# stefantaubert/waveglow

Hardware: AMD Instinct MI355X
Metric: audio samples/sec/GPU (22.05 kHz) WaveGlow-256 infer; real-time factor (higher is better)
Workload: dtype f16 MFMA operands, f32 accumulate/flow state, fp16 I/O; 1 GPU; configs[1]: 256ch WaveGlow.infer, batch=16/GPU mels 80x864, fp16 I/O, sigma=0.6; parallelism=utterance-sharded x1, no collective

## Files before the change

waveglow_amd/csrc/kernels.hip:

```cpp
#include "wg_common.h"

#include <cstdlib>
#include <type_traits>

namespace wg {

typedef _Float16 half8 __attribute__((ext_vector_type(8)));
typedef _Float16 half4 __attribute__((ext_vector_type(4)));
typedef float f32x16 __attribute__((ext_vector_type(16)));
typedef float f32x4 __attribute__((ext_vector_type(4)));

#define WG_GPTR(p) ((const __attribute__((address_space(1))) void*)(p))
#define WG_LPTR(p) ((__attribute__((address_space(3))) void*)(p))

__device__ __forceinline__ float load_io(const void* p, size_t i, int f16) {
  return f16 ? (float)((const _Float16*)p)[i] : ((const float*)p)[i];
}

__device__ __forceinline__ float gate_act(float u, float v) {
  const float e1 = __builtin_amdgcn_exp2f(__builtin_amdgcn_fmed3f(u, -60.0f, 60.0f));
  const float t = 1.0f + __builtin_amdgcn_exp2f(v);
  return (e1 - 1.0f) * __builtin_amdgcn_rcpf(fmaf(e1, t, t));
}

__device__ __forceinline__ void gate_act3(float u, float v, float& th, float& sg, float& ac) {
  const float e1 = __builtin_amdgcn_exp2f(__builtin_amdgcn_fmed3f(u, -60.0f, 60.0f));
  const float t = 1.0f + __builtin_amdgcn_exp2f(__builtin_amdgcn_fmed3f(v, -60.0f, 60.0f));
  const float r = __builtin_amdgcn_rcpf(fmaf(e1, t, t));
  ac = fmaf(e1, r, -r);
  sg = fmaf(e1, r, r);
  th = ac * t;
}

__device__ __forceinline__ void glds16(const void* sbase, unsigned voff, unsigned lds_addr) {
  unsigned keep;
  asm volatile("s_mov_b32 %0, m0\n\ts_mov_b32 m0, %3\n\ts_nop 2\n\tglobal_load_lds_dwordx4 %1, %2\n\ts_mov_b32 m0, %0"
               : "=&s"(keep) : "v"(voff), "s"(sbase), "s"(lds_addr) : "memory");
}
template <int OFF>
__device__ __forceinline__ void gload16(half8& dst, const void* sbase, unsigned voff) {
  asm volatile("s_nop 4\n\tglobal_load_dwordx4 %0, %1, %2 offset:%3" : "=v"(dst) : "v"(voff), "s"(sbase), "i"(OFF) : "memory");
}

#ifdef WG_STAMPS
#define WG_STAMP(i)                                                                              \
  do {                                                                                           \
    __builtin_amdgcn_sched_barrier(0);                                                           \
    unsigned long long _t;                                                                       \
    asm volatile("s_memtime %0\n\ts_waitcnt lgkmcnt(0)" : "=s"(_t)::"memory");                   \
    if (a.stamps && HAS_RES && tid == 0) a.stamps[(size_t)tile * 8 + (i)] = _t;                        \
    __builtin_amdgcn_sched_barrier(0);                                                           \
  } while (0)
#else
#define WG_STAMP(i) do {} while (0)
#endif

constexpr int kTilesPerWG = 2;


__device__ __forceinline__ void mfma16_acc(f32x4& c, const half8& a, const half8& b) {
  c = __builtin_amdgcn_mfma_f32_16x16x32_f16(a, b, c, 0, 0, 0);
}

template <int C> struct WnCfg {
  static constexpr int NW = (C >= 256) ? 8 : C / 32;
  static constexpr int BN = (C >= 512) ? 64 : 128;
};

template <int N> __device__ __forceinline__ void wait_vm() {
  asm volatile("s_waitcnt vmcnt(%0)" :: "i"(N) : "memory");
  __builtin_amdgcn_sched_barrier(0);
}

template <int C, int NW, int BN, bool HAS_RES, int TPW, int CX, int MODE = 0, int NTAPS = 3, bool HAS_COND = true, bool DEEP = false, bool M16 = false>
__global__ void __launch_bounds__(NW * 64) wn_layer_kernel(const WnLayerArgs a) {
  constexpr bool TR = MODE == 1;
  constexpr bool PLAIN = MODE >= 2;
  constexpr int MB = C / (32 * NW);
  constexpr int MT = PLAIN ? MB : 2 * MB;
  constexpr int NTHREADS = NW * 64;
  constexpr int NT = BN / 32;
  constexpr int CC = CX;
  constexpr int NKX = NTAPS * CC;
  constexpr int BT_BYTES = BN * 128;
  constexpr int ACT_ROW = 2 * C + 16;
  constexpr int K2 = C / 16;
  constexpr int NG = BN * 8 / NTHREADS;
  constexpr int NAH = MT * 2;
  constexpr bool DEFER = (MB == 1);
  static_assert(BN * 8 % NTHREADS == 0 && MB >= 1 && MB <= 2 && NKX >= 1 && (NTAPS == 1 || NTAPS == 3), "tile geometry");
  constexpr bool Q2L = !M16 && DEFER && !DEEP && (NG + NT - 1) / NT == 1 && NT >= NG + MT;
  static_assert(!M16 || (MODE == 0 && MB == 1 && DEFER && !DEEP && NT >= 2), "16x16x32 variant");
  constexpr bool A0G = MODE == 0 && CX == 1 && NTAPS == 1;
  static_assert(!DEEP || (MODE == 0 && DEFER && HAS_COND && MT <= NT && NG <= NT && ((NKX >= 4 && NKX % 2 == 0) || NKX == 1)), "deep prefetch variant");
  static_assert(MODE == 0 || (TPW == 1 && CX == ((MODE == 2 || MODE == 4) ? 2 : 1) * (C / 64)) || (MODE == 3 && CX == 1), "training variants");

  extern __shared__ __attribute__((aligned(16))) char smem[];
  char* const sB = smem;
  char* const sActs = MODE == 4 ? smem : smem + 2 * BT_BYTES;

  const int tid = threadIdx.x;
  const int wave = __builtin_amdgcn_readfirstlane(tid >> 6);
  int lane = tid & 63, ln = lane & 31, lh = lane >> 5;

  unsigned pvoff[NG];
  int pchunk[NG];
  int swB;
  int l15 = lane & 15, l4 = lane >> 4;
  unsigned a_voff;
  auto set_lane_ids = [&]() {
    int t = tid;
    asm volatile("" : "+v"(t));
    lane = t & 63;
    ln = lane & 31;
    lh = lane >> 5;
    swB = M16 ? (lane >> 1) & 7 : (ln >> 1) & 7;
    l15 = lane & 15;
    l4 = lane >> 4;
    a_voff = lane * 16;
#pragma unroll
    for (int i = 0; i < NG; ++i) {
      const int idx = i * NTHREADS + t;
      const int row = idx >> 3, pc = idx & 7;
      pchunk[i] = pc ^ ((row >> 1) & 7);
      pvoff[i] = row * 128 + (pchunk[i] << 4);
    }
  };
  set_lane_ids();
  const unsigned sB_addr = (unsigned)(size_t)WG_LPTR(sB);
  const int R = a.g.R, Rp = a.g.Rp, Fp = a.g.Fp, M = a.M;
  const int nK = NKX + (HAS_COND ? a.n_cond_steps : 0);
  const int mel_rows_per_utt = a.g.T + 6;

  auto xstep_src = [&](int p, int jt, int ks) -> const char* {
    const int tap = ks / CC, cc = ks - tap * CC;
    const int pp = p + (tap - NTAPS / 2) * a.dil;
    const int row = kRowPad + (pp & 31) * Rp + a.row0 + jt * BN + (pp >> 5);
    return (const char*)(a.x_tap + ((size_t)cc * R + row) * 64);
  };
  auto sp_src = [&](int p, int jt, int s_) -> const char* {
    const int row = kRowPad + p * Rp + a.row0 + jt * BN;
    return (const char*)(a.sp + ((size_t)s_ * R + row) * 64);
  };
  int mrow[NG];
  auto cond_voff = [&](int s, int i) -> unsigned {
    const int k0 = s * 64 + pchunk[i] * 8;
    const int j = (k0 >= M) + (k0 >= 2 * M) + (k0 >= 3 * M);
    return (unsigned)(((mrow[i] - j) * M + (k0 - j * M)) * 2);
  };
  auto stage_B_piece = [&](int p, int jt, int ks, int bufsel, int i) {
    const unsigned lds = __builtin_amdgcn_readfirstlane(sB_addr + bufsel * BT_BYTES + (i * NTHREADS + wave * 64) * 16);
    if constexpr (A0G) {
      if (ks < NKX) {
        const int row = (i * NTHREADS + tid) >> 3, lc = pchunk[i];
        const int pp = p + ((lc < 3 ? lc : 1) - 1) * a.dil;
        const unsigned prow = (unsigned)(kRowPad + (pp & 31) * Rp + a.row0 + jt * BN + (pp >> 5) + row);
        glds16(a.x_tap, prow * 128u + (lc < 3 ? 0u : (unsigned)lc * 16u), lds);
        return;
      }
    }
    if (ks < NKX) glds16(xstep_src(p, jt, ks), pvoff[i], lds);
    else if constexpr (MODE != 0) glds16(sp_src(p, jt, ks - NKX), pvoff[i], lds);
    else glds16(a.melT, cond_voff(ks - NKX, i), lds);
  };
  auto read_B = [&](const char* buf, int nt, int k16) -> half8 {
    const int n = nt * 32 + ln;
    const int c = (k16 * 2 + lh) ^ swB;
    return *(const half8*)(buf + n * 128 + c * 16);
  };
  auto read_B16 = [&](const char* buf, int g, int nt) -> half8 {
    const int n = (NT * (g & 1) + nt) * 16 + l15;
    const int c = (4 * (g >> 1) + l4) ^ swB;
    return *(const half8*)(buf + n * 128 + c * 16);
  };
  const char* wA1c_p = nullptr;
  auto load_Aq = [&](int ks, int g, int mt, half8& dst) {
    const char* base = ks < NKX ? (const char*)a.wA1 : wA1c_p;
    const int kl = ks < NKX ? ks : ks - NKX;
    const char* p = base + ((size_t)(2 * kl + (g >> 1)) * NW + wave) * (NAH * 1024) + (mt * 2 + (g & 1)) * 1024;
    gload16<0>(dst, p, a_voff);
  };
  auto load_A16 = [&](int ks, int s_, int m, half8& dst) {
    const char* base = ks < NKX ? (const char*)a.wA1 : wA1c_p;
    const int kl = ks < NKX ? ks : ks - NKX;
    gload16<0>(dst, base + ((size_t)(2 * kl + s_) * NW + wave) * (NAH * 1024) + m * 1024, a_voff);
  };
  int tile_b0 = 0;
  const bool fp_ge_bn = Fp >= BN;
  auto column_of = [&](int rr, int p, int& b, int& t) -> bool {
    int rem = rr - tile_b0 * Fp;
    b = tile_b0;
    if (fp_ge_bn) {
      if (rem >= Fp) { rem -= Fp; ++b; }
    } else {
      const int qd = rem / Fp;
      b += qd;
      rem -= qd * Fp;
    }
    const int fq = rem - a.g.Gf;
    t = fq * 32 + p;
    if (!(b < a.g.B && fq >= 0 && fq < a.g.F && t < a.g.L)) return false;
    return a.g.frames == nullptr || t < 32 * a.g.frames[b];
  };

  int tile, tile_end;
  const int tile_step = gridDim.x >> 3;
  int run_start, run_quarter = 0;
  {
    const int bid = blockIdx.x, ntl = a.n_tiles;
    const int xcd = bid & 7, idx = bid >> 3;
    const int qq = ntl >> 3, r = ntl & 7;
    const int start = xcd < r ? xcd * (qq + 1) : r * (qq + 1) + (xcd - r) * qq;
    tile_end = start + (xcd < r ? qq + 1 : qq);
    tile = start + idx;
    run_start = start;
    if (((tile_end - start) & 3) == 0) run_quarter = (tile_end - start) >> 2;
  }
  auto tile_of = [&](int t) { return run_quarter ? run_start + ((t - run_start) & 3) * run_quarter + ((t - run_start) >> 2) : t; };

  half8 q[4][MT];
  int par = 0;
  if (tile < tile_end) {
    const int t0 = tile_of(tile), p0 = t0 / a.tiles_per_phase;
#pragma unroll
    for (int i = 0; i < NG; ++i) stage_B_piece(p0, t0 - p0 * a.tiles_per_phase, 0, 0, i);
  }
  float* const sBias = (float*)(sActs + BN * ACT_ROW);
  if constexpr (!PLAIN) {
    for (int i = tid; i < 2 * C; i += NTHREADS) sBias[i] = a.bias1[i];
    if constexpr (HAS_RES)
      for (int i = tid; i < C; i += NTHREADS) sBias[2 * C + i] = a.bias2[i];
    uint4* const sW = (uint4*)(sBias + 3 * C);
    for (int i = tid; i < (C / 32) * 64; i += NTHREADS) sW[i] = ((const uint4*)a.wEs)[i];
  }
  __syncthreads();

#pragma unroll
  for (int it = 0; it < TPW; ++it, tile += tile_step) {
    if (tile >= tile_end) break;
    if (it > 0) set_lane_ids();
    const int tile_m = tile_of(tile);
    const int p = tile_m / a.tiles_per_phase;
    const int jt = tile_m - p * a.tiles_per_phase;
    const int rr0 = a.row0 + jt * BN;
    tile_b0 = rr0 / Fp;
    const int r0 = kRowPad + p * Rp + rr0;
    const int next_tile = tile + tile_step;
    wA1c_p = (const char*)a.wA1c + (MODE != 0 ? (size_t)0 : (size_t)p * (2 * a.n_cond_steps) * NW * (NAH * 1024));
    half8 Q[DEEP ? 2 : 1][4][MT];
    if constexpr (DEEP) {
#pragma unroll
      for (int g = 0; g < 4; ++g)
#pragma unroll
        for (int mt = 0; mt < MT; ++mt) load_Aq(0, g, mt, Q[0][g][mt]);
#pragma unroll
      for (int g = 0; g < 2; ++g)
#pragma unroll
        for (int mt = 0; mt < MT; ++mt) load_Aq(1, g, mt, Q[DEEP ? 1 : 0][g][mt]);
    } else {
#pragma unroll
      for (int g = 0; g < (Q2L || M16 ? 2 : 3); ++g)
#pragma unroll
        for (int mt = 0; mt < MT; ++mt) {
          if constexpr (M16) load_A16(0, 0, 2 * g + mt, q[g][mt]);
          else load_Aq(0, g, mt, q[g][mt]);
        }
    }
    if constexpr (MODE == 0) {
#pragma unroll
      for (int i = 0; i < NG; ++i) {
        int b, t;
        const int rr = rr0 + ((i * NTHREADS + tid) >> 3);
        const bool ok = column_of(rr, p, b, t);
        mrow[i] = ok ? 3 + b * mel_rows_per_utt + 3 + (t >> 5) : 3;
      }
    }
    unsigned vmask = 0;
#pragma unroll
    for (int nt = 0; nt < NT; ++nt) {
      int cb, ct;
      vmask |= column_of(rr0 + nt * 32 + ln, p, cb, ct) ? (1u << nt) : 0u;
    }
    WG_STAMP(0);
    f32x16 acc[MT][NT];
    f32x4 acc4[M16 ? MT : 1][M16 ? NT : 1][4];
    auto acc_at = [&](int mt, int nt, int e) -> float {
      if constexpr (M16) return acc4[mt][nt][e >> 2][e & 3];
      else return acc[mt][nt][e];
    };
#pragma unroll
    for (int mt = 0; mt < MT; ++mt) {
      f32x16 v;
      if constexpr (PLAIN) {
#pragma unroll
        for (int j = 0; j < 16; ++j) v[j] = 0.0f;
      } else {
        const int row0 = (mt < MB ? 0 : C) + (wave * MB + (mt < MB ? mt : mt - MB)) * 32;
        const float4* bp = (const float4*)(sBias + row0 + 4 * (M16 ? l4 : lh));
#pragma unroll
        for (int g = 0; g < 4; ++g) {
          const float4 q4 = bp[M16 ? 4 * (g >> 1) : 2 * g];
          v[4 * g] = q4.x; v[4 * g + 1] = q4.y; v[4 * g + 2] = q4.z; v[4 * g + 3] = q4.w;
        }
      }
#pragma unroll
      for (int nt = 0; nt < NT; ++nt) {
        if constexpr (M16) {
#pragma unroll
          for (int e = 0; e < 4; ++e) acc4[mt][nt][e] = f32x4{v[4 * e], v[4 * e + 1], v[4 * e + 2], v[4 * e + 3]};
        } else {
          acc[mt][nt] = v;
        }
      }
    }

    constexpr bool PIPE = !PLAIN && HAS_RES && MB == 1;
    constexpr bool RES_A0 = A0G && wn_res_a0(C);
    half8 a2r[PIPE ? K2 : 1];
    wait_vm<DEEP ? 3 * MT : 0>();
    __builtin_amdgcn_s_barrier();
    __builtin_amdgcn_sched_barrier(0);
    WG_STAMP(1);
    constexpr int LPS = (MT + NT - 1) / NT;
    constexpr int GPS = (NG + NT - 1) / NT;
    half8 bf[2][NT];
    constexpr bool PRIO = NW == 8 && ((BN == 128 && ((MODE == 0 && CX == C / 64) || MODE == 1)) || (C == 512 && MODE == 0 && CX == C / 64));
    auto prio_set = [&](int hi_grp) {
      if (hi_grp == 1)
        asm volatile("s_cmp_lt_u32 %0, 4\n\ts_cbranch_scc1 .Lpa%=\n\ts_setprio 1\n\ts_branch .Lpb%=\n.Lpa%=:\n\ts_setprio 0\n.Lpb%=:" :: "s"(wave) : "memory", "scc");
      else
        asm volatile("s_cmp_lt_u32 %0, 4\n\ts_cbranch_scc1 .Lpa%=\n\ts_setprio 0\n\ts_branch .Lpb%=\n.Lpa%=:\n\ts_setprio 1\n.Lpb%=:" :: "s"(wave) : "memory", "scc");
    };
    auto mfma_col = [&](int g, int nt) {
      if constexpr (M16) {
        const int t16 = NT * (g & 1) + nt;
#pragma unroll
        for (int m = 0; m < 4; ++m) {
          mfma16_acc(acc4[m >> 1][t16 >> 1][2 * (m & 1) + (t16 & 1)], q[2 * (g >> 1) + (m >> 1)][m & 1], bf[g & 1][nt]);
        }
      } else {
#pragma unroll
        for (int mt = 0; mt < MT; ++mt) {
          acc[mt][nt] = __builtin_amdgcn_mfma_f32_32x32x16_f16(q[g][mt], bf[g & 1][nt], acc[mt][nt], 0, 0, 0);
        }
      }
    };
    auto kstep = [&](auto more_tag, auto ncond_tag, auto first_tag, int ks) {
      constexpr bool more = decltype(more_tag)::value;
      constexpr bool ncond = decltype(ncond_tag)::value;
      constexpr bool first = decltype(first_tag)::value;
      const char* buf = sB + ((ks + par) & 1) * BT_BYTES;
      const char* src_next = nullptr;
      if constexpr (more && !ncond) src_next = xstep_src(p, jt, ks + 1);
      if constexpr (more && ncond && MODE != 0) src_next = sp_src(p, jt, ks + 1 - NKX);
      const unsigned lds_next = sB_addr + ((ks + 1 + par) & 1) * BT_BYTES + wave * 1024;
#pragma unroll
      for (int nt = 0; nt < NT; ++nt) bf[0][nt] = M16 ? read_B16(buf, 0, nt) : read_B(buf, nt, 0);
      __builtin_amdgcn_sched_barrier(0);
      auto dma_slot = [&](int nt) {
        if constexpr (more) {
#pragma unroll
          for (int i = nt * GPS; i < (nt + 1) * GPS && i < NG; ++i) {
            const unsigned lds = __builtin_amdgcn_readfirstlane(lds_next + i * NTHREADS * 16);
            if constexpr (ncond && MODE == 0) glds16(a.melT, cond_voff(ks + 1 - NKX, i), lds);
            else glds16(src_next, pvoff[i], lds);
          }
        }
      };
      if constexpr (PRIO) {
        prio_set(1);
        __builtin_amdgcn_sched_barrier(0);
      }
      if constexpr (DEFER) {
#pragma unroll
        for (int nt = 0; nt < NT; ++nt) {
          if constexpr (!first) mfma_col(3, nt);
          __builtin_amdgcn_sched_barrier(0);
          dma_slot(nt);
          if constexpr (Q2L) {
            if (nt >= NG && nt - NG < MT) load_Aq(ks, 2, nt - NG, q[2][nt - NG]);
          }
          __builtin_amdgcn_sched_barrier(0);
        }
      }
#pragma unroll
      for (int g = 0; g < (DEFER ? 3 : 4); ++g) {
        if constexpr (M16) {
          if (g == 0) wait_vm<more ? NG : 0>();
          if (g == 2) wait_vm<0>();
        } else {
        if (g == 1) wait_vm<more ? 2 * MT + NG : 2 * MT>();
        if (g == 2) wait_vm<Q2L ? (more ? 2 * MT : MT) : (more ? NG + 2 * MT : MT)>();
        if (g == 3) wait_vm<more ? 2 * MT : 0>();
        }
#pragma unroll
        for (int nt = 0; nt < NT; ++nt) {
          mfma_col(g, nt);
          __builtin_amdgcn_sched_barrier(0);
          if (g < 3) bf[(g + 1) & 1][nt] = M16 ? read_B16(buf, g + 1, nt) : read_B(buf, nt, g + 1);
          if (!DEFER && g == 0) dma_slot(nt);
          if constexpr (M16) {
            constexpr int LP16 = (4 + NT - 1) / NT;
            if (g == 0 || (g == 2 && more)) {
#pragma unroll
              for (int m = nt * LP16; m < (nt + 1) * LP16 && m < 4; ++m)
                load_A16(g == 0 ? ks : ks + 1, g == 0 ? 1 : 0, m, q[(g == 0 ? 2 : 0) + (m >> 1)][m & 1]);
            }
          } else if (g == 0 || more) {
#pragma unroll
            for (int mt = nt * LPS; mt < (nt + 1) * LPS && mt < MT; ++mt)
              load_Aq(g == 0 ? ks : ks + 1, (g + 3) & 3, mt, q[(g + 3) & 3][mt]);
          }
          if constexpr (PRIO) {
            if (g == 0 && nt == NT - 1) prio_set(0);
          }
          __builtin_amdgcn_sched_barrier(0);
        }
      }
      if constexpr (more) {
        if constexpr (DEFER && !Q2L && !M16) {
#pragma unroll
          for (int mt = 0; mt < MT; ++mt) load_Aq(ks + 1, 2, mt, q[2][mt]);
        }
        asm volatile("s_waitcnt vmcnt(%0) lgkmcnt(0)" :: "i"(M16 ? 4 : Q2L ? MT : 2 * MT) : "memory");
        __builtin_amdgcn_s_barrier();
        __builtin_amdgcn_sched_barrier(0);
      }
    };
    auto kstep_d = [&](auto par_tag, auto more_tag, auto more2_tag, auto ncond_tag, auto first_tag, int ks) {
      constexpr int P = DEEP ? decltype(par_tag)::value : 0, PO = DEEP ? 1 - P : 0;
      constexpr bool more = decltype(more_tag)::value, more2 = decltype(more2_tag)::value;
      constexpr bool ncond = decltype(ncond_tag)::value, first = decltype(first_tag)::value;
      const char* buf = sB + ((ks + par) & 1) * BT_BYTES;
      const char* src_next = nullptr;
      if constexpr (more && !ncond) src_next = xstep_src(p, jt, ks + 1);
      const unsigned lds_next = sB_addr + ((ks + 1 + par) & 1) * BT_BYTES + wave * 1024;
#pragma unroll
      for (int nt = 0; nt < NT; ++nt) bf[0][nt] = read_B(buf, nt, 0);
      __builtin_amdgcn_sched_barrier(0);
#pragma unroll
      for (int nt = 0; nt < NT; ++nt) {
        if constexpr (!first) {
#pragma unroll
          for (int mt = 0; mt < MT; ++mt)
            acc[mt][nt] = __builtin_amdgcn_mfma_f32_32x32x16_f16(Q[PO][3][mt], bf[1][nt], acc[mt][nt], 0, 0, 0);
        }
        __builtin_amdgcn_sched_barrier(0);
        if constexpr (more) {
          if (nt < NG) {
            const unsigned lds = __builtin_amdgcn_readfirstlane(lds_next + nt * NTHREADS * 16);
            if constexpr (ncond) glds16(a.melT, cond_voff(ks + 1 - NKX, nt), lds);
            else glds16(src_next, pvoff[nt], lds);
          }
          if (nt == NT - 1) {
#pragma unroll
            for (int mt = 0; mt < MT; ++mt) load_Aq(ks + 1, 2, mt, Q[PO][2][mt]);
          }
        }
        __builtin_amdgcn_sched_barrier(0);
      }
#pragma unroll
      for (int g = 0; g < 3; ++g) {
#pragma unroll
        for (int nt = 0; nt < NT; ++nt) {
#pragma unroll
          for (int mt = 0; mt < MT; ++mt)
            acc[mt][nt] = __builtin_amdgcn_mfma_f32_32x32x16_f16(Q[P][g][mt], bf[g & 1][nt], acc[mt][nt], 0, 0, 0);
          __builtin_amdgcn_sched_barrier(0);
          bf[(g + 1) & 1][nt] = read_B(buf, nt, g + 1);
          if (nt < MT) {
            if (g == 0 && more) load_Aq(ks + 1, 3, nt, Q[PO][3][nt]);
            if (g >= 1 && more2) load_Aq(ks + 2, g - 1, nt, Q[P][g - 1][nt]);
          }
          __builtin_amdgcn_sched_barrier(0);
        }
      }
      if constexpr (more) {
        asm volatile("s_waitcnt vmcnt(%0) lgkmcnt(0)" :: "i"(more2 ? 3 * MT : MT) : "memory");
        __builtin_amdgcn_s_barrier();
        __builtin_amdgcn_sched_barrier(0);
      }
    };
    if constexpr (DEEP) {
      using T_ = std::true_type;
      using F_ = std::false_type;
      using P0 = std::integral_constant<int, 0>;
      using P1 = std::integral_constant<int, 1>;
      if constexpr (NKX == 1) {
        kstep_d(P0{}, T_{}, T_{}, T_{}, T_{}, 0);
        kstep_d(P1{}, T_{}, T_{}, T_{}, F_{}, 1);
        kstep_d(P0{}, T_{}, T_{}, T_{}, F_{}, 2);
        kstep_d(P1{}, T_{}, T_{}, T_{}, F_{}, 3);
        kstep_d(P0{}, T_{}, F_{}, T_{}, F_{}, 4);
        kstep_d(P1{}, F_{}, F_{}, F_{}, F_{}, 5);
      } else {
        kstep_d(P0{}, T_{}, T_{}, F_{}, T_{}, 0);
#pragma clang loop unroll(disable)
        for (int ks = 1; ks < NKX - 1; ks += 2) {
          kstep_d(P1{}, T_{}, T_{}, F_{}, F_{}, ks);
          kstep_d(P0{}, T_{}, T_{}, F_{}, F_{}, ks + 1);
        }
        kstep_d(P1{}, T_{}, T_{}, T_{}, F_{}, NKX - 1);
        kstep_d(P0{}, T_{}, T_{}, T_{}, F_{}, NKX);
        kstep_d(P1{}, T_{}, T_{}, T_{}, F_{}, NKX + 1);
        kstep_d(P0{}, T_{}, T_{}, T_{}, F_{}, NKX + 2);
        kstep_d(P1{}, T_{}, F_{}, T_{}, F_{}, NKX + 3);
        kstep_d(P0{}, F_{}, F_{}, F_{}, F_{}, NKX + 4);
      }
      constexpr int PL = (NKX + 4) & 1;
      wait_vm<0>();
#pragma unroll
      for (int nt = 0; nt < NT; ++nt)
#pragma unroll
        for (int mt = 0; mt < MT; ++mt)
          acc[mt][nt] = __builtin_amdgcn_mfma_f32_32x32x16_f16(Q[DEEP ? PL : 0][3][mt], bf[1][nt], acc[mt][nt], 0, 0, 0);
    }
    if constexpr (!DEEP) {
      using T_ = std::true_type;
      using F_ = std::false_type;
      if constexpr (NKX == 1) {
        if constexpr (HAS_COND) kstep(T_{}, T_{}, T_{}, 0);
        else kstep(F_{}, F_{}, T_{}, 0);
      } else {
        kstep(T_{}, F_{}, T_{}, 0);
#pragma clang loop unroll(disable)
        for (int ks = 1; ks < NKX - 1; ++ks) kstep(T_{}, F_{}, F_{}, ks);
        if constexpr (HAS_COND) kstep(T_{}, T_{}, F_{}, NKX - 1);
        else kstep(F_{}, F_{}, F_{}, NKX - 1);
      }
      if constexpr (HAS_COND) {
#pragma clang loop unroll(disable)
        for (int ks = NKX; ks < nK - 1; ++ks) kstep(T_{}, T_{}, F_{}, ks);
        kstep(F_{}, F_{}, F_{}, nK - 1);
      }
    }
    if constexpr (DEFER && !DEEP) {
      wait_vm<0>();
#pragma unroll
      for (int nt = 0; nt < NT; ++nt) mfma_col(3, nt);
    }
    if constexpr (PRIO) asm volatile("s_setprio 0" ::: "memory");
    __builtin_amdgcn_sched_barrier(0);
    par = (par + nK) & 1;
// ... 204 lines not shown
      half8 idA[RES_A0 ? 1 : 2];
      if constexpr (RES_A0) {
        idA[0] = ((const half8*)a.wStA)[blk * 64 + laneo];
      } else {
        const int pr = 16 * ((lno >> 2) & 1) + 4 * (lno >> 3) + (lno & 3);
#pragma unroll
        for (int sx = 0; sx < 2; ++sx)
#pragma unroll
          for (int j = 0; j < 8; ++j) idA[sx][j] = (_Float16)((16 * sx + 8 * lho + j) == pr ? 1.0f : 0.0f);
      }
      half8 xr[RES_A0 ? 1 : 2];
      auto load_xr = [&](int nt) {
        if constexpr (RES_A0) {
          xr[0] = *(const half8*)(a.x_tap + ((size_t)r0 + nt * 32 + lno) * 64 + lho * 8);
        } else {
          const size_t row = (size_t)(blk >> 1) * R + r0 + nt * 32 + lno;
          const half8* xp = (const half8*)(a.x_in + row * 64 + (blk & 1) * 32 + lho * 8);
          xr[0] = xp[0];
          xr[1] = xp[2];
        }
      };
      load_xr(0);
      half8* const xo_base = (half8*)(a.x_out + ((size_t)(blk >> 1) * R + r0 + lno) * 64 + (blk & 1) * 32 + lho * 16);
      auto store_xout_half = [&](const f32x16& d, int nt, int hf) {
        if ((vmask >> nt) & 1u) {
          half8 qv;
#pragma unroll
          for (int r = 0; r < 8; ++r) qv[r] = (_Float16)d[8 * hf + r];
          xo_base[(size_t)nt * 32 * 8 + hf] = qv;
        }
      };
      __builtin_amdgcn_sched_barrier(0);
      auto phase = [&](auto c_tag) {
        constexpr int c = decltype(c_tag)::value;
        constexpr bool do_gate = c < NT, do_mm = c >= 1;
        f32x16 d2;
        if (do_mm) {
          const float4* bp = (const float4*)(sBias2 + blk * 32 + 4 * lho);
#pragma unroll
          for (int g = 0; g < 4; ++g) {
            const float4 b4 = bp[2 * g];
            d2[4 * g + 0] = b4.x;
            d2[4 * g + 1] = b4.y;
            d2[4 * g + 2] = b4.z;
            d2[4 * g + 3] = b4.w;
          }
          d2 = __builtin_amdgcn_mfma_f32_32x32x16_f16(idA[0], xr[0], d2, 0, 0, 0);
          if constexpr (!RES_A0) d2 = __builtin_amdgcn_mfma_f32_32x32x16_f16(idA[1], xr[1], d2, 0, 0, 0);
        }
        if (do_mm && c < NT) load_xr(c);
        if (c == NT - 1) es_prefetch();
        if (c == NT) es_compute();
        float e1[SL], den[SL], rc[SL];
        half8 o0, o1, th0, th1, sg0, sg1;
        auto stageA = [&](int e) {
          const int nt = c < NT ? c : 0;
          const float u = __builtin_amdgcn_fmed3f(acc_at(0, nt, e), -60.0f, 60.0f);
          e1[e] = __builtin_amdgcn_exp2f(u);
          den[e] = __builtin_amdgcn_exp2f(TR ? __builtin_amdgcn_fmed3f(acc_at(MB, nt, e), -60.0f, 60.0f) : acc_at(MB, nt, e));
        };
        auto stageB = [&](int e) {
          const float t = 1.0f + den[e];
          rc[e] = __builtin_amdgcn_rcpf(fmaf(e1[e], t, t));
          if constexpr (TR) den[e] = t;
        };
        auto stageC = [&](int e) {
          float v = fmaf(e1[e], rc[e], -rc[e]);
          asm volatile("" : "+v"(v));
          if (e < 8) o0[e] = (_Float16)v; else o1[e - 8] = (_Float16)v;
          if constexpr (TR) {
            float sg = fmaf(e1[e], rc[e], rc[e]), th = v * den[e];
            asm volatile("" : "+v"(sg), "+v"(th));
            if (e < 8) { sg0[e] = (_Float16)sg; th0[e] = (_Float16)th; } else { sg1[e - 8] = (_Float16)sg; th1[e - 8] = (_Float16)th; }
          }
        };
        bool save_ok = false;
        size_t save_off = 0;
        if constexpr (TR) {
          if (do_gate) {
            save_ok = (vmask >> c) & 1u;
            save_off = ((size_t)(blk >> 1) * R + r0 + c * 32 + lno) * 64 + (blk & 1) * 32 + lho * 16;
          }
        }
        static_assert(K2 <= SL, "one GEMM-2 MFMA per slot at most");
        half8 bq[K2];
        const int ntm = c >= 1 ? c - 1 : 0;
        auto k_of = [](int i) { return i * K2 / SL; };
        auto has_k = [&](int i) { return i >= 0 && i < SL && k_of(i) != k_of(i + 1); };
        if (do_gate) { stageA(0); stageA(1); stageB(0); }
        if (do_mm) {
          if (has_k(0)) bq[k_of(0)] = read_acts32(ntm, k_of(0));
          if (has_k(1)) bq[k_of(1)] = read_acts32(ntm, k_of(1));
        }
        __builtin_amdgcn_sched_barrier(0);
#pragma unroll
        for (int i = 0; i < SL; ++i) {
          if (do_mm) {
            if (has_k(i + 2)) bq[k_of(i + 2)] = read_acts32(ntm, k_of(i + 2));
            if (has_k(i)) d2 = __builtin_amdgcn_mfma_f32_32x32x16_f16(a2r[k_of(i)], bq[k_of(i)], d2, 0, 0, 0);
          }
          if (c == 0 && i < K2) a2r[i] = p2[(size_t)i * 64];
          if (do_gate) {
            if (i + 2 < SL) stageA(i + 2);
            if (i + 1 < SL) stageB(i + 1);
            if (i & 1) { stageC(i - 1); stageC(i); }
            if constexpr (M16) {
              if (i == 7) write_acts16(c, blk, 0, o0);
              if (i == SL - 1) write_acts16(c, blk, 1, o1);
            } else {
              if (i == 7) *(half8*)(acts_lane + c * 32 * ACT_ROW + blk * 64) = o0;
              if (i == SL - 1) *(half8*)(acts_lane + c * 32 * ACT_ROW + blk * 64 + 16) = o1;
            }
            if constexpr (TR) {
              if (i == 7 && save_ok) {
                *(half8*)(a.save_a + save_off) = o0;
                *(half8*)(a.save_t + save_off) = th0;
                *(half8*)(a.save_s + save_off) = sg0;
              }
              if (i == SL - 1 && save_ok) {
                *(half8*)(a.save_a + save_off + 8) = o1;
                *(half8*)(a.save_t + save_off + 8) = th1;
                *(half8*)(a.save_s + save_off + 8) = sg1;
              }
            }
          }
          __builtin_amdgcn_sched_barrier(0);
        }
        if (do_mm) {
          store_xout_half(d2, ntm, 0);
          store_xout_half(d2, ntm, 1);
        }
        if (do_gate) {
          asm volatile("s_waitcnt lgkmcnt(0)" ::: "memory");
          __builtin_amdgcn_s_barrier();
          asm volatile("" ::: "memory");
          __builtin_amdgcn_sched_barrier(0);
          if (c == 0) WG_STAMP(3);
          if (c == 1) WG_STAMP(5);
          if (c == 2) WG_STAMP(6);
          if (c == 3) WG_STAMP(7);
        }
      };
      phase(std::integral_constant<int, 0>{});
      phase(std::integral_constant<int, 1>{});
      if constexpr (NT >= 2) phase(std::integral_constant<int, 2>{});
      if constexpr (NT >= 3) phase(std::integral_constant<int, 3>{});
      if constexpr (NT >= 4) phase(std::integral_constant<int, 4>{});
      static_assert(NT <= 4, "phases are instantiated explicitly");
      WG_STAMP(4);
    }
    if constexpr (!PIPE) {
    if constexpr (HAS_RES) {
      if constexpr (RES_A0) {
#pragma unroll
        for (int nt = 0; nt < NT; ++nt) a0f[nt] = *(const half8*)(a.x_tap + ((size_t)r0 + nt * 32 + lno) * 64 + lho * 8);
#pragma unroll
        for (int mb = 0; mb < MB; ++mb) wst[mb] = ((const half8*)a.wStA)[(wave * MB + mb) * 64 + laneo];
      }
#pragma unroll
      for (int mb = 0; mb < MB; ++mb) {
        const int blk = wave * MB + mb;
        if constexpr (!RES_A0) {
#pragma unroll
          for (int nt = 0; nt < NT; ++nt) {
            const size_t row = (size_t)(blk >> 1) * R + r0 + nt * 32 + lno;
            const half8* xp = (const half8*)(a.x_in + row * 64 + (blk & 1) * 32 + lho * 16);
            xres[mb][nt][0] = xp[0];
            xres[mb][nt][1] = xp[1];
          }
        }
#pragma unroll
        for (int i = 0; i < PF; ++i) a2[mb][i] = p2[((size_t)mb * K2 + i) * 64];
      }
    }
    __builtin_amdgcn_sched_barrier(0);

#pragma unroll
    for (int mb = 0; mb < MB; ++mb) {
#pragma unroll
      for (int nt = 0; nt < NT; ++nt) {
        half8 o0, o1;
        if constexpr (TR) {
          half8 th0, th1, sg0, sg1;
#pragma unroll
          for (int r = 0; r < 8; ++r) {
            float th, sg, ac;
            gate_act3(acc[mb][nt][r], acc[MB + mb][nt][r], th, sg, ac);
            o0[r] = (_Float16)ac; th0[r] = (_Float16)th; sg0[r] = (_Float16)sg;
            gate_act3(acc[mb][nt][8 + r], acc[MB + mb][nt][8 + r], th, sg, ac);
            o1[r] = (_Float16)ac; th1[r] = (_Float16)th; sg1[r] = (_Float16)sg;
          }
          int cb, ct;
          if (column_of(rr0 + nt * 32 + lno, p, cb, ct)) {
            const int blk = wave * MB + mb;
            const size_t off = ((size_t)(blk >> 1) * R + r0 + nt * 32 + lno) * 64 + (blk & 1) * 32 + lho * 16;
            *(half8*)(a.save_a + off) = o0; *(half8*)(a.save_a + off + 8) = o1;
            *(half8*)(a.save_t + off) = th0; *(half8*)(a.save_t + off + 8) = th1;
            *(half8*)(a.save_s + off) = sg0; *(half8*)(a.save_s + off + 8) = sg1;
          }
        } else {
#pragma unroll
          for (int r = 0; r < 8; ++r) {
            o0[r] = (_Float16)gate_act(acc_at(mb, nt, r), acc_at(MB + mb, nt, r));
            o1[r] = (_Float16)gate_act(acc_at(mb, nt, 8 + r), acc_at(MB + mb, nt, 8 + r));
          }
        }
        if constexpr (M16) {
          write_acts16(nt, wave * MB + mb, 0, o0);
          write_acts16(nt, wave * MB + mb, 1, o1);
        } else {
          char* ap = acts_lane + nt * 32 * ACT_ROW + (wave * MB + mb) * 64;
          *(half8*)(ap) = o0;
          *(half8*)(ap + 16) = o1;
        }
      }
    }
    __syncthreads();
    __builtin_amdgcn_sched_barrier(0);
    WG_STAMP(3);

    if constexpr (HAS_RES) {
#pragma unroll
      for (int mb = 0; mb < MB; ++mb) {
        const float* bp = a.bias2 + (wave * MB + mb) * 32 + 4 * lho;
        float bv[16];
#pragma unroll
        for (int r = 0; r < 16; ++r) bv[r] = bp[(r & 3) + 8 * (r >> 2)];
#pragma unroll
        for (int nt = 0; nt < NT; ++nt) {
          if constexpr (RES_A0) {
#pragma unroll
            for (int r = 0; r < 16; ++r) acc2[mb][nt][r] = bv[r];
            acc2[mb][nt] = __builtin_amdgcn_mfma_f32_32x32x16_f16(wst[mb], a0f[nt], acc2[mb][nt], 0, 0, 0);
          } else {
#pragma unroll
            for (int r = 0; r < 8; ++r) {
              acc2[mb][nt][r] = (float)xres[mb][nt][0][r] + bv[r];
              acc2[mb][nt][8 + r] = (float)xres[mb][nt][1][r] + bv[8 + r];
            }
          }
        }
      }
    }

    }


    if constexpr (kWesEarly && !PIPE) es_prefetch();

    if constexpr (HAS_RES && !PIPE) {
      half8 bq[2][NT];
#pragma unroll
      for (int nt = 0; nt < NT; ++nt) bq[0][nt] = read_acts32(nt, 0);
#pragma unroll
      for (int k = 0; k < K2; ++k) {
        if (k + 1 < K2) {
#pragma unroll
          for (int nt = 0; nt < NT; ++nt) bq[(k + 1) & 1][nt] = read_acts32(nt, k + 1);
        }
#pragma unroll
        for (int mb = 0; mb < MB; ++mb) {
          const half8 af = a2[mb][k % PF];
          if (k + PF < K2) a2[mb][k % PF] = p2[((size_t)mb * K2 + k + PF) * 64];
#pragma unroll
          for (int nt = 0; nt < NT; ++nt)
            acc2[mb][nt] = __builtin_amdgcn_mfma_f32_32x32x16_f16(af, bq[k & 1][nt], acc2[mb][nt], 0, 0, 0);
        }
      }
    }

    if constexpr (!PIPE) {
      WG_STAMP(4);
      if constexpr (!kWesEarly) es_prefetch();
      es_compute();
    }

    if constexpr (!PIPE) WG_STAMP(5);
    if constexpr (HAS_RES && !PIPE) {
#pragma unroll
      for (int nt = 0; nt < NT; ++nt) {
        int cb, ct;
        if (column_of(rr0 + nt * 32 + lno, p, cb, ct)) {
#pragma unroll
          for (int mb = 0; mb < MB; ++mb) {
            const int blk = wave * MB + mb;
            half8 o0, o1;
#pragma unroll
            for (int r = 0; r < 8; ++r) {
              o0[r] = (_Float16)acc2[mb][nt][r];
              o1[r] = (_Float16)acc2[mb][nt][8 + r];
            }
            const size_t row = (size_t)(blk >> 1) * R + r0 + nt * 32 + lno;
            half8* xp = (half8*)(a.x_out + row * 64 + (blk & 1) * 32 + lho * 16);
            xp[0] = o0;
            xp[1] = o1;
          }
        }
      }
    }
    if constexpr (!PIPE) WG_STAMP(6);
    }
    __builtin_amdgcn_sched_barrier(0);
  }
}

template <int C, int BN, bool HAS_RES, int TPW, int CX, int MODE = 0, int NTAPS = 3, bool HAS_COND = true, bool DEEP = false>
static hipError_t launch_wn_tttt(const WnLayerArgs& a, hipStream_t s) {
  constexpr int NW = WnCfg<C>::NW;
  constexpr bool M16 = wn_frag16(C, BN) && MODE == 0 && !DEEP;
  if (M16 != (a.frag16 != 0)) return hipErrorInvalidValue;
  if (MODE == 0 && CX == 1 && NTAPS == 1 && wn_res_a0(C) && HAS_RES && !a.wStA) return hipErrorInvalidValue;
  constexpr int smem = MODE == 4 ? (BN * (2 * C + 16) > 2 * BN * 128 ? BN * (2 * C + 16) : 2 * BN * 128)
                                 : 2 * BN * 128 + (MODE >= 2 ? 0 : BN * (2 * C + 16) + 3 * C * 4 + (C / 32) * 1024);
  static bool attr_done_dev[64] = {};
  int cur_dev = 0;
  if (hipGetDevice(&cur_dev) != hipSuccess || cur_dev < 0 || cur_dev >= 64) cur_dev = 0;
  bool& attr_done = attr_done_dev[cur_dev];
  if (!attr_done) {
    hipError_t e = hipFuncSetAttribute((const void*)wn_layer_kernel<C, NW, BN, HAS_RES, TPW, CX, MODE, NTAPS, HAS_COND, DEEP, M16>,
                                       hipFuncAttributeMaxDynamicSharedMemorySize, smem);
    if (e != hipSuccess) return e;
    attr_done = true;
  }
  const int per_label = ((a.n_tiles + 7) / 8 + TPW - 1) / TPW;
  const int grid = 8 * per_label;
  hipLaunchKernelGGL((wn_layer_kernel<C, NW, BN, HAS_RES, TPW, CX, MODE, NTAPS, HAS_COND, DEEP, M16>), dim3(grid), dim3(NW * 64), smem, s, a);
  return hipGetLastError();
}
template <int C, int BN, bool HAS_RES, int TPW>
static hipError_t launch_wn_ttt(const WnLayerArgs& a, hipStream_t s) {
  if constexpr (C == 256 && BN == 64 && TPW == 1) {
    const char* e = getenv("WG_DISABLE_DEEP");
    if (a.n_cond_steps == 5 && !(e && *e == '1')) {
      if (a.a0_fold) return launch_wn_tttt<C, BN, HAS_RES, TPW, 1, 0, 1, true, true>(a, s);
      return launch_wn_tttt<C, BN, HAS_RES, TPW, C / 64, 0, 3, true, true>(a, s);
    }
  }
  if (a.a0_fold) return a.x_chunks_per_tap == 1 ? launch_wn_tttt<C, BN, HAS_RES, TPW, 1, 0, 1>(a, s) : hipErrorInvalidValue;
  return launch_wn_tttt<C, BN, HAS_RES, TPW, C / 64>(a, s);
}
template <int C, int BN, bool HAS_RES>
static hipError_t launch_wn_tt(const WnLayerArgs& a, hipStream_t s) {
  const int ncu = a.n_cu > 0 ? a.n_cu : 1;
  const int rounds1 = (a.n_tiles + ncu - 1) / ncu;
  const int rounds2 = ((a.n_tiles + kTilesPerWG - 1) / kTilesPerWG + ncu - 1) / ncu * kTilesPerWG;
  if (a.n_tiles >= 2 * kTilesPerWG * ncu && rounds2 <= rounds1) return launch_wn_ttt<C, BN, HAS_RES, kTilesPerWG>(a, s);
  return launch_wn_ttt<C, BN, HAS_RES, 1>(a, s);
}
template <int C>
static hipError_t launch_wn_t(const WnLayerArgs& a, int bn, hipStream_t s) {
  if (bn == 64) return a.has_res ? launch_wn_tt<C, 64, true>(a, s) : launch_wn_tt<C, 64, false>(a, s);
  if constexpr (WnCfg<C>::BN == 128) {
    if (bn == 128) return a.has_res ? launch_wn_tt<C, 128, true>(a, s) : launch_wn_tt<C, 128, false>(a, s);
  }
  return hipErrorInvalidValue;
}

int wn_block_n(int C) {
  switch (C) {
    case 64: return WnCfg<64>::BN;
    case 128: return WnCfg<128>::BN;
    case 256: return WnCfg<256>::BN;
    case 512: return WnCfg<512>::BN;
  }
  return 0;
}
int wn_waves(int C) {
  switch (C) {
    case 64: return WnCfg<64>::NW;
    case 128: return WnCfg<128>::NW;
    case 256: return WnCfg<256>::NW;
    case 512: return WnCfg<512>::NW;
  }
  return 0;
}

template <int C>
static hipError_t launch_wn_train_t(const WnLayerArgs& a, int bn, hipStream_t s) {
  if (bn == 64) return a.has_res ? launch_wn_tttt<C, 64, true, 1, C / 64, 1>(a, s) : launch_wn_tttt<C, 64, false, 1, C / 64, 1>(a, s);
  if constexpr (WnCfg<C>::BN == 128) {
    if (bn == 128) return a.has_res ? launch_wn_tttt<C, 128, true, 1, C / 64, 1>(a, s) : launch_wn_tttt<C, 128, false, 1, C / 64, 1>(a, s);
  }
  return hipErrorInvalidValue;
}
hipError_t launch_wn_layer_train(const WnLayerArgs& a, int C, int bn, hipStream_t s) {
  if (!a.sp || !a.save_t || !a.save_s || !a.save_a || a.x_chunks_per_tap != C / 64) return hipErrorInvalidValue;
  switch (C) {
    case 64: return launch_wn_train_t<64>(a, bn, s);
    case 128: return launch_wn_train_t<128>(a, bn, s);
    case 256: return launch_wn_train_t<256>(a, bn, s);
    case 512: return launch_wn_train_t<512>(a, bn, s);
  }
  return hipErrorInvalidValue;
}

template <int C>
static hipError_t launch_wn_plain_t(const WnLayerArgs& a, int kind, int bn, hipStream_t s) {
  constexpr int CCH = C / 64;
  if constexpr (WnCfg<C>::BN == 128) {
    if (bn == 128) {
      if (kind == 2) return launch_wn_tttt<C, 128, false, 1, 2 * CCH, 2, 3, false>(a, s);
      if (kind == 4) return launch_wn_tttt<C, 128, false, 1, 2 * CCH, 4, 3, false>(a, s);
      if (a.x_chunks_per_tap == 1 && a.n_cond_steps == 0) return launch_wn_tttt<C, 128, false, 1, 1, 3, 1, false>(a, s);
      return launch_wn_tttt<C, 128, false, 1, CCH, 3, 1, true>(a, s);
    }
  }
  if (bn != 64) return hipErrorInvalidValue;
  if (kind == 2) return launch_wn_tttt<C, 64, false, 1, 2 * CCH, 2, 3, false>(a, s);
  if (kind == 4) return launch_wn_tttt<C, 64, false, 1, 2 * CCH, 4, 3, false>(a, s);
  if (a.x_chunks_per_tap == 1 && a.n_cond_steps == 0) return launch_wn_tttt<C, 64, false, 1, 1, 3, 1, false>(a, s);
  return launch_wn_tttt<C, 64, false, 1, CCH, 3, 1, true>(a, s);
}
hipError_t launch_wn_plain(const WnLayerArgs& a, int C, int kind, int bn, hipStream_t s) {
  if ((kind != 2 && kind != 3 && kind != 4) || !a.out0 || !a.x_tap || (kind == 3 && (!a.in0 || !a.in1))) return hipErrorInvalidValue;
  if ((kind == 2 || kind == 4) && (a.x_chunks_per_tap != 2 * (C / 64) || a.n_cond_steps != 0)) return hipErrorInvalidValue;
  if (kind == 4 && (!a.wat_prev || !a.gout || !a.t_prev || !a.s_prev || !a.dpre_prev)) return hipErrorInvalidValue;
  if (kind == 3 && !((a.x_chunks_per_tap == 1 && a.n_cond_steps == 0) || (a.x_chunks_per_tap == C / 64 && a.n_cond_steps == 1 && a.sp)))
    return hipErrorInvalidValue;
  switch (C) {
    case 64: return launch_wn_plain_t<64>(a, kind, bn, s);
    case 128: return launch_wn_plain_t<128>(a, kind, bn, s);
    case 256: return launch_wn_plain_t<256>(a, kind, bn, s);
    case 512: return launch_wn_plain_t<512>(a, kind, bn, s);
  }
  return hipErrorInvalidValue;
}

hipError_t launch_wn_layer(const WnLayerArgs& a, int C, int bn, hipStream_t s) {
  switch (C) {
    case 64: return launch_wn_t<64>(a, bn, s);
    case 128: return launch_wn_t<128>(a, bn, s);
    case 256: return launch_wn_t<256>(a, bn, s);
    case 512: return launch_wn_t<512>(a, bn, s);
  }
  return hipErrorInvalidValue;
}

__global__ void __launch_bounds__(256) mel_pack_kernel(const MelPackArgs a) {
  const int rows_per_utt = a.T + 6;
  const size_t n = (size_t)(3 + a.B * rows_per_utt) * a.M;
  for (size_t idx = (size_t)blockIdx.x * 256 + threadIdx.x; idx < n; idx += (size_t)gridDim.x * 256) {
    const int i = (int)(idx % a.M);
    const int row = (int)(idx / a.M) - 3;
    float v = 0.0f;
    if (row >= 0) {
      const int b = row / rows_per_utt, f = row - b * rows_per_utt - 3;
      if (f >= 0 && f < (a.frames ? a.frames[b] : a.T)) v = load_io(a.mel, ((size_t)b * a.M + i) * a.T + f, a.io_f16);
    }
    a.melT[idx] = (_Float16)v;
  }
}

__global__ void __launch_bounds__(256) zero_fill_kernel(uint4* __restrict__ p, size_t n16) {
  for (size_t i = (size_t)blockIdx.x * 256 + threadIdx.x; i < n16; i += (size_t)gridDim.x * 256)
    p[i] = make_uint4(0u, 0u, 0u, 0u);
}
hipError_t launch_zero_fill(void* p, size_t bytes, hipStream_t s) {
  if (((size_t)p & 15) || (bytes & 15)) return hipErrorInvalidValue;
  size_t blocks = (bytes / 16 + 255) / 256;
  if (blocks > 4096) blocks = 4096;
  if (blocks < 1) blocks = 1;
  hipLaunchKernelGGL(zero_fill_kernel, dim3((unsigned)blocks), dim3(256), 0, s, (uint4*)p, bytes / 16);
  return hipGetLastError();
}

hipError_t launch_mel_pack(const MelPackArgs& a, hipStream_t s) {
  const size_t n = (size_t)(3 + a.B * (a.T + 6)) * a.M;
  unsigned blocks = (unsigned)((n + 255) / 256);
  if (blocks > 4096) blocks = 4096;
  hipLaunchKernelGGL(mel_pack_kernel, dim3(blocks), dim3(256), 0, s, a);
  return hipGetLastError();
}

__global__ void __launch_bounds__(256) cond_fold_kernel(const float* __restrict__ w_cond, const float* __restrict__ w_up,
                                                        _Float16* __restrict__ out, int C, int NW, int M, int up_kernel,
                                                        float tanh_scale, float sigm_scale, int frag16) {
  __shared__ float sW[64][33];
  __shared__ float sU[32][81];
  const int p = blockIdx.x >> 2, j = blockIdx.x & 3;
  const int m0 = blockIdx.y * 64;
  const int l = blockIdx.z;
  const int NS = M * 8, MB = C / (32 * NW), MT = 2 * MB;
  const int tid = threadIdx.x;
  float acc[20];
#pragma unroll
  for (int e = 0; e < 20; ++e) acc[e] = 0.0f;
  const int per_thread = (64 * M + 255) / 256;
  for (int s0 = 0; s0 < NS; s0 += 32) {
    for (int e = tid; e < 64 * 32; e += 256) {
      const int mm = e >> 5, ss = e & 31;
      sW[mm][ss] = w_cond[((size_t)(2 * C * l + m0 + mm)) * NS + s0 + ss];
    }
    for (int e = tid; e < 32 * M; e += 256) {
      const int ss = e / M, i = e - ss * M;
      const int sch = s0 + ss, o = sch >> 3, g = sch & 7;
      sU[ss][i] = w_up[((size_t)i * M + o) * up_kernel + 8 * p + g + 256 * j];
    }
    __syncthreads();
    for (int e = 0; e < per_thread; ++e) {
      const int idx = e * 256 + tid;
      if (idx < 64 * M) {
        const int mm = idx / M, i = idx - mm * M;
        float v = acc[e];
#pragma unroll 8
        for (int ss = 0; ss < 32; ++ss) v = fmaf(sW[mm][ss], sU[ss][i], v);
        acc[e] = v;
      }
    }
    __syncthreads();
  }
  const int n_half = 2 * (M / 16);
  for (int e = 0; e < per_thread; ++e) {
    const int idx = e * 256 + tid;
    if (idx >= 64 * M) continue;
    const int mm = idx / M, i = idx - mm * M;
    const int m = m0 + mm;
    const bool tanh_row = m < C;
    const int ch = tanh_row ? m : m - C;
    const int blk = ch >> 5, r = ch & 31;
    const int w = blk / MB, mt = (tanh_row ? 0 : MB) + (blk - w * MB);
    const int kk = j * M + i;
    const int u = kk >> 5, k2 = (kk >> 4) & 1, hh = (kk >> 3) & 1, jj = kk & 7;
    const _Float16 val = (_Float16)(acc[e] * (tanh_row ? tanh_scale : sigm_scale));
    if (frag16) {
      const int m16 = 2 * (tanh_row ? 0 : 1) + (r >> 4), kg = (kk >> 3) & 3;
      const size_t f16 = (((size_t)(l * kPhases + p) * n_half + u) * NW + w) * 4 + m16;
      out[(f16 * 64 + kg * 16 + (r & 15)) * 8 + jj] = val;
      continue;
    }
    const size_t frag = ((((size_t)(l * kPhases + p) * n_half + u) * NW + w) * MT + mt) * 2 + k2;
    out[(frag * 64 + hh * 32 + r) * 8 + jj] = val;
  }
}

hipError_t launch_cond_fold(const float* w_cond, const float* w_up, _Float16* out, int C, int NW, int M, int n_layers,
                            int up_kernel, float tanh_scale, float sigm_scale, int frag16, hipStream_t s) {
  if (M > 80 || M % 16 || (frag16 && C != 32 * NW)) return hipErrorInvalidValue;
  dim3 grid(kPhases * 4, 2 * C / 64, n_layers);
  hipLaunchKernelGGL(cond_fold_kernel, grid, dim3(256), 0, s, w_cond, w_up, out, C, NW, M, up_kernel, tanh_scale,
                     sigm_scale, frag16);
  return hipGetLastError();
}

template <int FL_ROWS>
__device__ __forceinline__ void start_rows(const float4* s_a0, size_t row0, size_t nrows, int L, const RowGeom& g,
                                           const float* __restrict__ wstart, const float* __restrict__ bstart, int C, int h,
                                           _Float16* x) {
  const int tid = threadIdx.x;
  const int g8 = tid & 7;
  unsigned prow[8];
  unsigned ok = 0;
#pragma unroll
  for (int it = 0; it < 8; ++it) {
    const int rl = it * (FL_ROWS / 8) + (tid >> 3);
    const size_t row = row0 + rl;
    prow[it] = 0;
    if (row >= nrows) continue;
    const unsigned r32 = (unsigned)row;
    const int b = (int)(r32 / (unsigned)L), t = (int)(r32 - (unsigned)b * (unsigned)L);
    if (g.frames != nullptr && t >= 32 * g.frames[b]) continue;
    prow[it] = (unsigned)kRowPad + (unsigned)(t & 31) * (unsigned)g.Rp + (unsigned)b * (unsigned)g.Fp + (unsigned)g.Gf + (unsigned)(t >> 5);
    ok |= 1u << it;
  }
  for (int cc = 0; cc < C / 64; ++cc) {
    const int P0 = cc * 64 + g8 * 8;
    float w[8][4], bs[8];
#pragma unroll
    for (int e = 0; e < 8; ++e) {
      bs[e] = bstart[P0 + e];
#pragma unroll
      for (int j = 0; j < 4; ++j) w[e][j] = (j < h) ? wstart[(P0 + e) * h + j] : 0.0f;
    }
#pragma unroll
    for (int it = 0; it < 8; ++it) {
      if (!((ok >> it) & 1u)) continue;
      const int rl = it * (FL_ROWS / 8) + (tid >> 3);
      const float4 a0 = s_a0[rl];
      half8 o;
#pragma unroll
      for (int e = 0; e < 8; ++e)
        o[e] = (_Float16)fmaf(w[e][3], a0.w, fmaf(w[e][2], a0.z, fmaf(w[e][1], a0.y, fmaf(w[e][0], a0.x, bs[e]))));
      *(half8*)(x + ((size_t)cc * g.R + prow[it]) * 64 + g8 * 8) = o;
    }
  }
}

template <int FL_ROWS>
__global__ void __launch_bounds__(FL_ROWS) flow_kernel(const FlowArgs a) {
  __shared__ float4 s_a0[FL_ROWS];
  const int L = a.g.L;
  const size_t nrows = (size_t)a.g.B * L;
  const size_t row0 = (size_t)blockIdx.x * FL_ROWS;
  const int tid = threadIdx.x;

  {
    const size_t row = row0 + tid;
    if (row < nrows) {
      const unsigned r32 = (unsigned)row;
      const int b = (int)(r32 / (unsigned)L), t = (int)(r32 - (unsigned)b * (unsigned)L);
      const bool pad_row = a.g.frames != nullptr && t >= 32 * a.g.frames[b];
      float zn[kMaxGroup];
#pragma unroll
      for (int c = 0; c < kMaxGroup; ++c) zn[c] = 0.0f;
      if (a.direction == 0) {
        if (a.first) {
#pragma unroll
          for (int c = 0; c < kMaxGroup; ++c)
            if (c < a.c_next)
              zn[c] = a.sigma * load_io(a.z_extra, ((size_t)b * a.c_next + c) * L + t, a.io_f16);
        } else {
          float z[kMaxGroup], o[kMaxGroup], v[kMaxGroup], y[kMaxGroup];
          const float4* zp = (const float4*)(a.Z + row * 8);
          const float4* op = (const float4*)(a.out + row * 8);
          float4 z0 = zp[0], z1 = zp[1], o0 = op[0], o1 = op[1];
          z[0] = z0.x; z[1] = z0.y; z[2] = z0.z; z[3] = z0.w; z[4] = z1.x; z[5] = z1.y; z[6] = z1.z; z[7] = z1.w;
          o[0] = o0.x; o[1] = o0.y; o[2] = o0.z; o[3] = o0.w; o[4] = o1.x; o[5] = o1.y; o[6] = o1.z; o[7] = o1.w;
          const int h = a.h_in, c = a.c_in;
#pragma unroll
          for (int j = 0; j < kMaxGroup; ++j) {
            float num = z[j], den = 1.0f;
#pragma unroll
            for (int q = 0; q < 4; ++q)
              if (j >= h && j - h == q) { num = z[j] - o[q]; den = expf(o[j]); }
            v[j] = (j < c) ? num / den : 0.0f;
          }
#pragma unroll
          for (int r = 0; r < kMaxGroup; ++r) {
            float s = 0.0f;
#pragma unroll
            for (int cc = 0; cc < kMaxGroup; ++cc)
              if (r < c && cc < c) s = fmaf(a.winv[r * c + cc], v[cc], s);
            y[r] = s;
          }
          const int ne = a.n_extra;
#pragma unroll
          for (int e = 0; e < kMaxGroup; ++e) {
            float val = 0.0f;
            if (e < ne) val = a.sigma * load_io(a.z_extra, ((size_t)b * ne + e) * L + t, a.io_f16);
#pragma unroll
            for (int r = 0; r < kMaxGroup; ++r)
              if (e >= ne && e - ne == r) val = y[r];
            zn[e] = val;
          }
        }
        if (a.last) {
          if (pad_row) {
// ... 173 lines not shown
```

Before: 78.78 million samples/s.

## Add persistent resident-workgroup tile walk for 256-channel WN layer kernel

Adds a RESIDENT variant of the WN layer kernel that wraps the per-workgroup tile loop in an outer do-while. Each workgroup keeps walking tiles until its range is exhausted, and the grid is sized to about one workgroup per CU instead of one per tile pair. The launcher picks this path by default for C=256, BN=128 when there are enough tiles and the tail wave is not tiny, and an environment variable can force or disable it. The aim is to amortize the per-workgroup prologue (bias/weight staging into LDS, first B staging) and reduce launch and tail overhead. The risk is worse load balance or lost latency hiding from fewer resident waves.

```diff
diff --git a/waveglow_amd/csrc/kernels.hip b/waveglow_amd/csrc/kernels.hip
--- a/waveglow_amd/csrc/kernels.hip
+++ b/waveglow_amd/csrc/kernels.hip
@@ -72,7 +72,8 @@
   __builtin_amdgcn_sched_barrier(0);
 }
 
-template <int C, int NW, int BN, bool HAS_RES, int TPW, int CX, int MODE = 0, int NTAPS = 3, bool HAS_COND = true, bool DEEP = false, bool M16 = false>
+template <int C, int NW, int BN, bool HAS_RES, int TPW, int CX, int MODE = 0, int NTAPS = 3, bool HAS_COND = true, bool DEEP = false, bool M16 = false,
+          bool RESIDENT = false>
 __global__ void __launch_bounds__(NW * 64) wn_layer_kernel(const WnLayerArgs a) {
   constexpr bool TR = MODE == 1;
   constexpr bool PLAIN = MODE >= 2;
@@ -93,6 +94,7 @@
   static_assert(!M16 || (MODE == 0 && MB == 1 && DEFER && !DEEP && NT >= 2), "16x16x32 variant");
   constexpr bool A0G = MODE == 0 && CX == 1 && NTAPS == 1;
   static_assert(!DEEP || (MODE == 0 && DEFER && HAS_COND && MT <= NT && NG <= NT && ((NKX >= 4 && NKX % 2 == 0) || NKX == 1)), "deep prefetch variant");
+  static_assert(!RESIDENT || (MODE == 0 && TPW == kTilesPerWG && !DEEP), "resident tile walk");
   static_assert(MODE == 0 || (TPW == 1 && CX == ((MODE == 2 || MODE == 4) ? 2 : 1) * (C / 64)) || (MODE == 3 && CX == 1), "training variants");
 
   extern __shared__ __attribute__((aligned(16))) char smem[];
@@ -235,10 +237,12 @@
   }
   __syncthreads();
 
+#pragma clang loop unroll(disable)
+  do {
 #pragma unroll
   for (int it = 0; it < TPW; ++it, tile += tile_step) {
     if (tile >= tile_end) break;
-    if (it > 0) set_lane_ids();
+    if (RESIDENT || it > 0) set_lane_ids();
     const int tile_m = tile_of(tile);
     const int p = tile_m / a.tiles_per_phase;
     const int jt = tile_m - p * a.tiles_per_phase;
@@ -1049,10 +1053,11 @@
     }
     __builtin_amdgcn_sched_barrier(0);
   }
-}
-
-template <int C, int BN, bool HAS_RES, int TPW, int CX, int MODE = 0, int NTAPS = 3, bool HAS_COND = true, bool DEEP = false>
-static hipError_t launch_wn_tttt(const WnLayerArgs& a, hipStream_t s) {
+  } while (RESIDENT && tile < tile_end);
+}
+
+template <int C, int BN, bool HAS_RES, int TPW, int CX, int MODE = 0, int NTAPS = 3, bool HAS_COND = true, bool DEEP = false, bool RESIDENT = false>
+static hipError_t launch_wn_tttt(const WnLayerArgs& a, hipStream_t s, int resident_wgs = 0) {
   constexpr int NW = WnCfg<C>::NW;
   constexpr bool M16 = wn_frag16(C, BN) && MODE == 0 && !DEEP;
   if (M16 != (a.frag16 != 0)) return hipErrorInvalidValue;
@@ -1064,18 +1069,19 @@
   if (hipGetDevice(&cur_dev) != hipSuccess || cur_dev < 0 || cur_dev >= 64) cur_dev = 0;
   bool& attr_done = attr_done_dev[cur_dev];
   if (!attr_done) {
-    hipError_t e = hipFuncSetAttribute((const void*)wn_layer_kernel<C, NW, BN, HAS_RES, TPW, CX, MODE, NTAPS, HAS_COND, DEEP, M16>,
+    hipError_t e = hipFuncSetAttribute((const void*)wn_layer_kernel<C, NW, BN, HAS_RES, TPW, CX, MODE, NTAPS, HAS_COND, DEEP, M16, RESIDENT>,
                                        hipFuncAttributeMaxDynamicSharedMemorySize, smem);
     if (e != hipSuccess) return e;
     attr_done = true;
   }
-  const int per_label = ((a.n_tiles + 7) / 8 + TPW - 1) / TPW;
+  if (RESIDENT != (resident_wgs > 0)) return hipErrorInvalidValue;
+  const int per_label = RESIDENT ? resident_wgs : ((a.n_tiles + 7) / 8 + TPW - 1) / TPW;
   const int grid = 8 * per_label;
-  hipLaunchKernelGGL((wn_layer_kernel<C, NW, BN, HAS_RES, TPW, CX, MODE, NTAPS, HAS_COND, DEEP, M16>), dim3(grid), dim3(NW * 64), smem, s, a);
+  hipLaunchKernelGGL((wn_layer_kernel<C, NW, BN, HAS_RES, TPW, CX, MODE, NTAPS, HAS_COND, DEEP, M16, RESIDENT>), dim3(grid), dim3(NW * 64), smem, s, a);
   return hipGetLastError();
 }
-template <int C, int BN, bool HAS_RES, int TPW>
-static hipError_t launch_wn_ttt(const WnLayerArgs& a, hipStream_t s) {
+template <int C, int BN, bool HAS_RES, int TPW, bool RESIDENT = false>
+static hipError_t launch_wn_ttt(const WnLayerArgs& a, hipStream_t s, int resident_wgs = 0) {
   if constexpr (C == 256 && BN == 64 && TPW == 1) {
     const char* e = getenv("WG_DISABLE_DEEP");
     if (a.n_cond_steps == 5 && !(e && *e == '1')) {
@@ -1083,12 +1089,25 @@
       return launch_wn_tttt<C, BN, HAS_RES, TPW, C / 64, 0, 3, true, true>(a, s);
     }
   }
-  if (a.a0_fold) return a.x_chunks_per_tap == 1 ? launch_wn_tttt<C, BN, HAS_RES, TPW, 1, 0, 1>(a, s) : hipErrorInvalidValue;
-  return launch_wn_tttt<C, BN, HAS_RES, TPW, C / 64>(a, s);
+  if (a.a0_fold)
+    return a.x_chunks_per_tap == 1 ? launch_wn_tttt<C, BN, HAS_RES, TPW, 1, 0, 1, true, false, RESIDENT>(a, s, resident_wgs) : hipErrorInvalidValue;
+  return launch_wn_tttt<C, BN, HAS_RES, TPW, C / 64, 0, 3, true, false, RESIDENT>(a, s, resident_wgs);
 }
 template <int C, int BN, bool HAS_RES>
 static hipError_t launch_wn_tt(const WnLayerArgs& a, hipStream_t s) {
   const int ncu = a.n_cu > 0 ? a.n_cu : 1;
+  {
+    const char* e = getenv("WG_RESIDENT");
+    const int forced = e && *e ? atoi(e) : -1;
+    const int per_label_tiles = (a.n_tiles + 7) / 8;
+    int wgs = 0;
+    if (forced > 0) wgs = (forced + 7) / 8;
+    else if (forced < 0 && C == 256 && BN == 128 && a.n_tiles >= 2 * ncu && !(a.n_tiles % ncu > 0 && 4 * (a.n_tiles % ncu) < ncu)) {
+      const int by_tiles = (per_label_tiles + kTilesPerWG - 1) / kTilesPerWG, by_cus = (ncu + 7) / 8;
+      wgs = by_tiles < by_cus ? by_tiles : by_cus;
+    }
+    if (wgs > 0) return launch_wn_ttt<C, BN, HAS_RES, kTilesPerWG, true>(a, s, wgs);
+  }
   const int rounds1 = (a.n_tiles + ncu - 1) / ncu;
   const int rounds2 = ((a.n_tiles + kTilesPerWG - 1) / kTilesPerWG + ncu - 1) / ncu * kTilesPerWG;
   if (a.n_tiles >= 2 * kTilesPerWG * ncu && rounds2 <= rounds1) return launch_wn_ttt<C, BN, HAS_RES, kTilesPerWG>(a, s);
```

Measured after the change: 79.69 million samples/s (median of 6 runs). +1.1%, better.
